# fwilliams/point-cloud-utils

Hardware: AMD Instinct MI355X
Metric: query-points/s, Chamfer 1M-vs-1M fp32 (higher is better)
Workload: dtype f32

## Files before the change

### point_cloud_utils_amd/csrc/search.h

```cpp
#pragma once
#include "pcu_types.h"
#include "grid.h"
#include "reduce.h"

namespace pcu {

template <typename T>
struct SearchArgs {
    const GridParams<T>* gp;
    const Pt4<T>* ref;
    const T* ref_xyz;
    const unsigned* cell_start;
    const Pt4<T>* qsorted;
    const T* q_xyz; const int* q_idx;
    const int* ref_idx;
    int lean;
    const int* qlist;
    const int* qcount_dev;
    int nq;
    int R;
    const int* qlist2; const int* qcount2_dev; int R2;
    unsigned n_ref;
    unsigned lane_max_cand;
    float skew_far;
// ... 286 lines not shown
        if (!active || outside) return;
    }

    const int ccx = grid_cell(g, 0, q.x), ccy = grid_cell(g, 1, q.y), ccz = grid_cell(g, 2, q.z);
    const int x0 = max(ccx - 1, 0), x1 = min(ccx + 1, Gx - 1);
    const int y0 = max(ccy - 1, 0), y1 = min(ccy + 1, Gy - 1);
    const int z0 = max(ccz - 1, 0), z1 = min(ccz + 1, Gz - 1);

    T bd[K];
    int bi[K];
#pragma unroll
    for (int i = 0; i < K; ++i) { bd[i] = Limits<T>::max_v; bi[i] = 0x7fffffff; }
    bool tie = false;

    unsigned rs[9], re[9];
#pragma unroll
    for (int j = 0; j < 9; ++j) {
        const int cy = ccy + kRowOy[j], cz = ccz + kRowOz[j];
        const bool ok = cy >= 0 && cy < Gy && cz >= 0 && cz < Gz;
        const int lo = row_run_lo(Gx, grid_row(Gy, ok ? cy : ccy, ok ? cz : ccz), x0, x1);
        rs[j] = a.cell_start[lo];
        const unsigned e = a.cell_start[lo + (x1 - x0 + 1)];
        re[j] = ok ? e : rs[j];
    }
    constexpr int kGroup = 4;
    const char* const base = reinterpret_cast<const char*>(a.ref);
    const unsigned sentinel = a.n_ref;
    unsigned total = 0;
#pragma unroll
    for (int j = 0; j < 9; ++j) total += re[j] - rs[j];
    const bool defer = total > a.lane_max_cand;
    T rlb[9];
    row_lower_bounds(g, q, ccy, ccz, rlb);
    constexpr int kBuf = K > 1 ? PCU_KBUF : 1;
    __shared__ T s_bd[kBuf][kBlock];
    __shared__ int s_bi[kBuf][kBlock];
    const int tid = threadIdx.x;
    int cnt = 0;
    auto flush = [&]() {
        int mx = cnt;
#pragma unroll
        for (int o = 32; o > 0; o >>= 1) mx = max(mx, __shfl_xor(mx, o, 64));
        for (int i = 0; i < mx; ++i)
            if (i < cnt) offer<T, K>(s_bd[i][tid], s_bi[i][tid], bd, bi, tie);
        cnt = 0;
    };
#pragma unroll
    for (int j = 0; j < 9; ++j) {
        if (K > 1 && __any(cnt >= kBuf / 2)) flush();
        const unsigned e = (defer || bd[K - 1] < rlb[j]) ? rs[j] : re[j];
        auto load_group = [&](unsigned p, Pt4<T> (&c)[kGroup]) {
#pragma unroll
            for (int u = 0; u < kGroup; ++u) {
                const unsigned idx = (p + u < e) ? p + u : sentinel;
                c[u] = *reinterpret_cast<const Pt4<T>*>(base + (size_t)(idx * (unsigned)sizeof(Pt4<T>)));
            }
        };
        auto eval_group = [&](const Pt4<T> (&c)[kGroup]) {
            if (K == 1) {
#pragma unroll
                for (int u = 0; u < kGroup; ++u) offer<T, K>(dist2(q, c[u]), (int)c[u].idx, bd, bi, tie);
            } else {
#pragma unroll
                for (int u = 0; u < kGroup; ++u) {
                    const T d = dist2(q, c[u]);
                    tie = tie || (d == bd[K - 1]);
                    if (d < bd[K - 1]) { s_bd[cnt][tid] = d; s_bi[cnt][tid] = (int)c[u].idx; ++cnt; }
                }
                if (__any(cnt > kBuf - kGroup)) flush();
            }
        };
        if (K > 1) {
            unsigned p = rs[j];
            if (p < e) {
                Pt4<T> ca[kGroup], cb[kGroup];
                load_group(p, ca);
                for (;;) {
                    p += kGroup;
                    load_group(p < e ? p : sentinel, cb);
                    eval_group(ca);
                    if (!(p < e)) break;
                    p += kGroup;
                    load_group(p < e ? p : sentinel, ca);
                    eval_group(cb);
                    if (!(p < e)) break;
                }
            }
        } else {
            for (unsigned p = rs[j]; p < e; p += kGroup) {
                Pt4<T> c[kGroup];
                load_group(p, c);
                eval_group(c);
            }
        }
    }
    if (K > 1) flush();

    finish_lane<T, K>(a, g, q, qpos, x0, x1, y0, y1, z0, z1, bd, bi, tie, true, defer);
}

__device__ __forceinline__ int cell_of_query(const GridParams<float>& g, const int axis, const float v) {
    const float t = (v - g.org[axis]) * g.inv_h;
    return (int)__builtin_amdgcn_fmed3f(t, 0.f, (float)(g.G[axis] - 1));
}
__device__ __forceinline__ int cell_of_query(const GridParams<double>& g, const int axis, const double v) { return grid_cell(g, axis, v); }
template <typename T> struct K1Group { static constexpr int n = 4; };
struct __attribute__((packed, aligned(4))) CellStart4 { unsigned v[4]; };
typedef float f32x2 __attribute__((ext_vector_type(2)));
__device__ __forceinline__ float min4(float a, float b, float c, float d) { return __builtin_fminf(__builtin_fminf(__builtin_fminf(a, b), c), d); }
__device__ __forceinline__ double min4(double a, double b, double c, double d) { return __builtin_fmin(__builtin_fmin(a, b), __builtin_fmin(c, d)); }

__device__ __forceinline__ unsigned lb_pack(float lb) { return __float_as_uint(lb) >> 16; }
__device__ __forceinline__ unsigned lb_pack(double lb) { const double v = lb * (1.0 - 1e-6); return __float_as_uint((float)(v < 1e38 ? v : 1e38)) >> 16; }
template <typename T> __device__ __forceinline__ T lb_unpack(unsigned b) { return (T)__uint_as_float(b << 16); }


template <typename T> struct __attribute__((packed, aligned(4))) Group12 { T v[12]; };
template <unsigned REC> __device__ __forceinline__ unsigned rec_bytes(unsigned i) {
    static_assert(REC == 12u || REC == 24u || REC == 16u || REC == 32u, "record sizes of the candidate streams");
    if (REC == 16u) return i << 4;
    if (REC == 32u) return i << 5;
    unsigned r; const unsigned t = REC == 12u ? i << 2 : i << 3;
    if (REC == 12u) asm("v_lshl_add_u32 %0, %1, 3, %2" : "=v"(r) : "v"(i), "v"(t));
    else asm("v_lshl_add_u32 %0, %1, 4, %2" : "=v"(r) : "v"(i), "v"(t));
    return r;
}
__device__ __forceinline__ unsigned mad24(unsigned a, unsigned b, unsigned c) { unsigned r; asm("v_mad_u32_u24 %0, %1, %2, %3" : "=v"(r) : "v"(a), "v"(b), "v"(c)); return r; }

template <typename T> struct GroupEval;
template <> struct GroupEval<float> {
    static constexpr unsigned kRec = 12u;
    typedef Group12<float> Raw;
    static __device__ __forceinline__ Raw load(const char* base, unsigned off) { return *reinterpret_cast<const Raw*>(base + (size_t)off); }
    static __device__ __forceinline__ void dists(const Raw& g, const Pt4<float>& q, float (&d)[4]) {
        const f32x2 qxy = {q.x, q.y}, qzx = {q.z, q.x}, qyz = {q.y, q.z};
        f32x2 p0 = qxy - f32x2{g.v[0], g.v[1]}, p1 = qzx - f32x2{g.v[2], g.v[3]}, p2 = qyz - f32x2{g.v[4], g.v[5]};
        f32x2 p3 = qxy - f32x2{g.v[6], g.v[7]}, p4 = qzx - f32x2{g.v[8], g.v[9]}, p5 = qyz - f32x2{g.v[10], g.v[11]};
        p0 = p0 * p0; p1 = p1 * p1; p2 = p2 * p2; p3 = p3 * p3; p4 = p4 * p4; p5 = p5 * p5;
        d[0] = (p0.x + p0.y) + p1.x; d[1] = (p1.y + p2.x) + p2.y; d[2] = (p3.x + p3.y) + p4.x; d[3] = (p4.y + p5.x) + p5.y;
    }
};
template <> struct GroupEval<double> {
    static constexpr unsigned kRec = 24u;
    typedef Group12<double> Raw;
    static __device__ __forceinline__ Raw load(const char* base, unsigned off) { return *reinterpret_cast<const Raw*>(base + (size_t)off); }
    static __device__ __forceinline__ void dists(const Raw& g, const Pt4<double>& q, double (&d)[4]) {
#pragma unroll
        for (int u = 0; u < 4; ++u) { const double dx = q.x - g.v[3 * u], dy = q.y - g.v[3 * u + 1], dz = q.z - g.v[3 * u + 2]; d[u] = ((dx * dx) + (dy * dy)) + (dz * dz); }
    }
};
template <typename T> struct BitsOf;
template <> struct BitsOf<float> { typedef unsigned type; static __device__ __forceinline__ unsigned of(float v) { return __float_as_uint(v); } static __device__ __forceinline__ float back(unsigned b) { return __uint_as_float(b); } };
template <> struct BitsOf<double> { typedef unsigned long long type; static __device__ __forceinline__ unsigned long long of(double v) { return (unsigned long long)__double_as_longlong(v); } static __device__ __forceinline__ double back(unsigned long long b) { return __longlong_as_double((long long)b); } };
template <typename T, bool EARLY, int FUSE>
__device__ __forceinline__ void search1_flat_body(const SearchArgs<T>& a, const int nq_arg, const int bid, const int nblk, bool& f_ok, T& f_v, long long& f_key) {
    typedef GroupEval<T> GE;
    __shared__ uint2 s_rng[8][kBlock];
    const int per = nblk >> 3;
    const int vb = (bid & 7) * per + (bid >> 3);
    const int tid = threadIdx.x;
    const int nq = a.qcount_dev ? *a.qcount_dev : nq_arg;
    if (vb * kBlock >= nq) return;
    const GridParams<T> g = uniform_params(*a.gp);
    if (const int hl = index_not_ready(a, g)) { if (vb == 0 && tid == 0) a.skew_flag[kLargeFlag] = hl; return; }
    const float ssq = uniform((float)g.sumsq);
    if (a.skew_limit > 0.f && (ssq > a.skew_limit || ssq < a.skew_lo)) { if (vb == 0 && tid == 0) *a.skew_flag = ssq > a.skew_far ? 2 : 1; return; }
    const int t = vb * kBlock + tid;
    if (t >= nq) return;
    constexpr bool valid = true;
    auto query_pos = [&]() { return a.qlist ? a.qlist[t] : t; };
    Pt4<T> q;
    {
        struct __attribute__((packed, aligned(4))) Q3 { T v[3]; };
        const Q3 c = *reinterpret_cast<const Q3*>(a.q_xyz + 3 * (size_t)query_pos());
        q.x = c.v[0]; q.y = c.v[1]; q.z = c.v[2];
        q.idx = 0;
    }
    static_assert(FUSE != FUSE_ARGMAX, "fused arg-max calls take the value-only program (FUSE_MAXVAL)");
    constexpr bool VALUE_ONLY = FUSE == FUSE_SUM || FUSE == FUSE_MAXVAL;
    const int Gx = g.G[0], Gy = g.G[1], Gz = g.G[2];
    const int ccx = cell_of_query(g, 0, q.x), ccy = cell_of_query(g, 1, q.y), ccz = cell_of_query(g, 2, q.z);
    constexpr unsigned kRec = GE::kRec;
    constexpr int kG = K1Group<T>::n;
    const char* const base = reinterpret_cast<const char*>(a.ref_xyz);
    const unsigned cand_cap = a.lane_max_cand < 65535u ? a.lane_max_cand : 65535u;
    T best = Limits<T>::max_v;
    unsigned boff = 0xffffffffu, toff = 0xffffffffu;
    bool tie = false, tie2 = false;
#define PCU_K1_EVAL(RAW, OFF)                                                                                \
    {                                                                                                        \
        T d_[4]; GE::dists((RAW), q, d_);                                                                    \
        const T m_ = min4(d_[0], d_[1], d_[2], d_[3]);                                                       \
        const bool eq_ = m_ == best, lt_ = m_ < best;                                                        \
        tie2 = !lt_ && (tie2 || (tie && eq_));                                                               \
        tie = !lt_ && (tie || eq_);                                                                          \
        toff = eq_ ? (OFF) : toff;                                                                           \
        best = lt_ ? m_ : best;                                                                              \
        boff = lt_ ? (OFF) : boff;                                                                           \
    }
    const bool hasxl = ccx > 0, hasxh = ccx < Gx - 1;
    const bool odd0 = ((ccy ^ ccz) & 1) != 0, zodd = (ccz & 1) != 0;
    const bool hasA = (odd0 && hasxh) || (!odd0 && hasxl), hasB = (odd0 && hasxl) || (!odd0 && hasxh);
    const unsigned Gx4 = (unsigned)Gx << 2;
    const unsigned xe4 = (unsigned)ccx << 2, xo4 = (unsigned)(Gx - 1 - ccx) << 2;
    const unsigned xS4 = odd0 ? xo4 : xe4, xR4 = odd0 ? xe4 : xo4;
    const int yS = zodd ? Gy - 1 - ccy : ccy, sS = zodd ? -1 : 1;
    const int row0 = (int)mad24((unsigned)ccz, (unsigned)Gy, (unsigned)yS);
    const int flip = (Gy - 1 - yS) - yS;
    const int rowM = row0 + flip - Gy, rowP = row0 + flip + Gy;
    const bool okyM = ccy > 0, okyP = ccy < Gy - 1, okzM = ccz > 0, okzP = ccz < Gz - 1;
    const char* const tbase = reinterpret_cast<const char*>(a.cell_start) - 4;
    auto row_table = [&](int j, bool& ok) {
        const int oy = kRowOy[j], oz = kRowOz[j];
        ok = (oy == 0 || (oy < 0 ? okyM : okyP)) && (oz == 0 || (oz < 0 ? okzM : okzP));
        const int rr = oz == 0 ? row0 + oy * sS : (oz < 0 ? rowM : rowP) - oy * sS;
        const unsigned row = (unsigned)(ok ? rr : row0);
        return *reinterpret_cast<const CellStart4*>(tbase + (size_t)(__umul24(row, Gx4) + (((oy + oz) & 1) == 0 ? xS4 : xR4)));
    };
    bool okj[9];
    CellStart4 tb[9];
    tb[0] = row_table(0, okj[0]);
    if (EARLY) {
#pragma unroll
        for (int j = 1; j < 9; ++j) tb[j] = row_table(j, okj[j]);
    }
    const unsigned c_s = hasA ? tb[0].v[0] : tb[0].v[1], c_e = hasB ? tb[0].v[3] : tb[0].v[2];
    const unsigned cnt0 = c_e - c_s;
    bool defer = cnt0 > cand_cap;
    {
        const unsigned o0 = rec_bytes<kRec>(c_s);
        const unsigned o1 = (defer || !valid) ? o0 : rec_bytes<kRec>(c_e);
        for (unsigned off = o0; off < o1; off += (unsigned)kG * kRec) { const typename GE::Raw raw = GE::load(base, off); PCU_K1_EVAL(raw, off) }
    }
    if (!EARLY) {
#pragma unroll
        for (int j = 1; j < 9; ++j) tb[j] = row_table(j, okj[j]);
    }
    const T shrink = (T)1 - (T)4 * Limits<T>::eps;
    T mxl = q.x - face_below(g, 0, ccx); mxl = mxl > (T)0 ? mxl * shrink : (T)0;
    T mxh = face_above(g, 0, ccx) - q.x; mxh = mxh > (T)0 ? mxh * shrink : (T)0;
    const T mxl2 = mxl * mxl, mxh2 = mxh * mxh;
    const T mA2 = odd0 ? mxh2 : mxl2, mB2 = odd0 ? mxl2 : mxh2;
    T my2[3], mz2[3];
    {
        T m;
        my2[0] = (T)0; mz2[0] = (T)0;
        m = q.y - face_below(g, 1, ccy); m = m > (T)0 ? m * shrink : (T)0; my2[1] = m * m;
        m = face_above(g, 1, ccy) - q.y; m = m > (T)0 ? m * shrink : (T)0; my2[2] = m * m;
        m = q.z - face_below(g, 2, ccz); m = m > (T)0 ? m * shrink : (T)0; mz2[1] = m * m;
        m = face_above(g, 2, ccz) - q.z; m = m > (T)0 ? m * shrink : (T)0; mz2[2] = m * m;
    }
    unsigned total = cnt0;
    int n = 0;
#pragma unroll
    for (int j = 1; j < 9; ++j) {
        const int oy = kRowOy[j], oz = kRowOz[j];
        const T ry = my2[oy == 0 ? 0 : (oy < 0 ? 1 : 2)], rz = mz2[oz == 0 ? 0 : (oz < 0 ? 1 : 2)];
        const bool same = ((oy + oz) & 1) == 0;
        const T mF2 = same ? mA2 : mB2, mL2 = same ? mB2 : mA2;
        const bool hasF = same ? hasA : hasB, hasL = same ? hasB : hasA;
        const T rlb = oy == 0 ? rz : (oz == 0 ? ry : ry + rz);
        const T bF = oy == 0 ? mF2 + rz : (oz == 0 ? mF2 + ry : (mF2 + ry) + rz), bL = oy == 0 ? mL2 + rz : (oz == 0 ? mL2 + ry : (mL2 + ry) + rz);
        const bool cutF = !hasF || best < bF, cutL = !hasL || best < bL;
        const unsigned s_run = cutF ? tb[j].v[1] : tb[j].v[0], e_run = cutL ? tb[j].v[2] : tb[j].v[3];
        const bool take = okj[j] && !defer && !(best < rlb) && e_run > s_run;
        s_rng[n][tid] = make_uint2(rec_bytes<kRec>(s_run), ((e_run - s_run) << 16) | lb_pack(rlb));
        n += take ? 1 : 0;
        total += take ? e_run - s_run : 0u;
    }
    if (total > cand_cap) { defer = true; n = 0; }
    const int own = tid;
    int r = 0;
    unsigned off = 0, end = 0;
    bool live = false;
    auto next_run = [&]() {
        live = false;
        while (r < n) {
            const uint2 e = s_rng[r][own];
            ++r;
            if (!(best < lb_unpack<T>(e.y & 0xffffu))) { off = e.x; end = e.x + __umul24(e.y >> 16, kRec); live = true; break; }
        }
    };
    next_run();
    const unsigned sent_off = a.n_ref * kRec;
#ifndef PCU_ADOPT_T
#define PCU_ADOPT_T 3
#endif
    if (VALUE_ONLY) {
        constexpr int kAdoptCap = 160;
        constexpr int kOwn = PCU_ADOPT_T;
        typedef typename BitsOf<T>::type Bits;
        __shared__ unsigned s_aitem[kBlock / 64][kAdoptCap];
        __shared__ Bits s_abest[kBlock / 64][64];
        const int lane_ = tid & 63, wave_ = tid >> 6;
        constexpr unsigned kStep = (unsigned)kG * kRec;
        if (live) {
            typename GE::Raw g0 = GE::load(base, off);
#pragma unroll
            for (int it = 0; it < kOwn; ++it) {
                const unsigned coff = off;
                off += kStep;
                if (off >= end) next_run();
                typename GE::Raw g1;
                if (it + 1 < kOwn) g1 = GE::load(base, live ? off : sent_off);
                PCU_K1_EVAL(g0, coff)
                if (!live) break;
                if (it + 1 < kOwn) g0 = g1;
            }
        }
        if (__ballot(true) == ~0ull && a.n_ref < (1u << 26)) {
            unsigned c = 0;
            if (live) {
                c = (end - off + kStep - 1u) / kStep;
                for (int rr = r; rr < n; ++rr) { const uint2 e = s_rng[rr][own]; if (!(best < lb_unpack<T>(e.y & 0xffffu))) c += ((e.y >> 16) + (unsigned)kG - 1u) / (unsigned)kG; }
            }
            unsigned inc = c;
#pragma unroll
            for (int o = 1; o < 64; o <<= 1) { const unsigned u = (unsigned)__shfl_up((int)inc, o, 64); if (lane_ >= o) inc += u; }
            const unsigned W = (unsigned)__shfl((int)inc, 63, 64);
            if (W != 0u && W <= (unsigned)kAdoptCap) {
                unsigned slot = inc - c;
                const unsigned tag = (unsigned)lane_ << 26;
                if (c) {
                    for (unsigned o = off; o < end; o += kStep) { s_aitem[wave_][slot] = (o / kRec) | tag; ++slot; }
                    for (int rr = r; rr < n; ++rr) {
                        const uint2 e = s_rng[rr][own];
                        if (!(best < lb_unpack<T>(e.y & 0xffffu))) {
                            const unsigned r0 = e.x / kRec, r1 = r0 + (e.y >> 16);
                            for (unsigned o = r0; o < r1; o += (unsigned)kG) { s_aitem[wave_][slot] = o | tag; ++slot; }
                        }
                    }
                }
                s_abest[wave_][lane_] = BitsOf<T>::of(best);
                __builtin_amdgcn_fence(__ATOMIC_RELEASE, "wavefront");
                __builtin_amdgcn_wave_barrier();
                __builtin_amdgcn_fence(__ATOMIC_ACQUIRE, "wavefront");
                for (unsigned wb = 0; wb < W; wb += 64u) {
                    const unsigned w_ = wb + (unsigned)lane_;
                    const bool in_ = w_ < W;
                    const unsigned it_ = in_ ? s_aitem[wave_][in_ ? w_ : 0u] : 0u;
                    const int ql = in_ ? (int)(it_ >> 26) : lane_;
                    const typename GE::Raw g1 = GE::load(base, in_ ? rec_bytes<kRec>(it_ & 0x03ffffffu) : sent_off);
                    Pt4<T> qq; qq.x = __shfl(q.x, ql, 64); qq.y = __shfl(q.y, ql, 64); qq.z = __shfl(q.z, ql, 64); qq.idx = 0;
                    T d_[4]; GE::dists(g1, qq, d_);
                    const T m_ = min4(d_[0], d_[1], d_[2], d_[3]);
                    if (in_) atomicMin(&s_abest[wave_][ql], BitsOf<T>::of(m_));
                }
                __builtin_amdgcn_fence(__ATOMIC_RELEASE, "wavefront");
                __builtin_amdgcn_wave_barrier();
                __builtin_amdgcn_fence(__ATOMIC_ACQUIRE, "wavefront");
                best = BitsOf<T>::back(s_abest[wave_][lane_]);
                live = false;
            }
        }
    }
    if (live) {
        typename GE::Raw ga = GE::load(base, off), gb;
        for (;;) {
            unsigned coff = off;
            off += (unsigned)kG * kRec;
            if (off >= end) next_run();
            gb = GE::load(base, live ? off : sent_off);
            PCU_K1_EVAL(ga, coff)
            if (!live) break;
            coff = off;
            off += (unsigned)kG * kRec;
            if (off >= end) next_run();
            ga = GE::load(base, live ? off : sent_off);
            PCU_K1_EVAL(gb, coff)
            if (!live) break;
        }
    }
    T lb;
    {
        const T smax = g.slack[0] > g.slack[1] ? (g.slack[0] > g.slack[2] ? g.slack[0] : g.slack[2]) : (g.slack[1] > g.slack[2] ? g.slack[1] : g.slack[2]);
        const T mag = ((fabs(g.org[0]) + fabs(g.org[1])) + fabs(g.org[2])) + (T)(Gx + Gy + Gz + 3) * g.h + smax;
        const T hq = (g.h - (T)2 * smax) - (T)16 * Limits<T>::eps * mag;
        const T hs = hq > (T)0 ? hq * shrink : (T)0;
        lb = hs * hs;
    }
    if (__ballot(valid && !defer && !(best < lb)) != 0ull) {
        const int cx0 = max(ccx - 1, 0), cx1 = min(ccx + 1, Gx - 1);
        const int cy0 = max(ccy - 1, 0), cy1 = min(ccy + 1, Gy - 1), cz0 = max(ccz - 1, 0), cz1 = min(ccz + 1, Gz - 1);
        lb = face_lower_bound_inner(g, q.x, q.y, q.z, cx0, cx1, cy0, cy1, cz0, cz1);
        unsigned long long todo = __ballot(valid && !defer && !(best < lb));
        if (todo && __popcll(todo) <= 4 && __ballot(true) == ~0ull) {
            const int lane_ = tid & 63;
            while (todo) {
                const int l = __ffsll((long long)todo) - 1;
                todo &= todo - 1;
                Pt4<T> sq;
                sq.x = __shfl(q.x, l, 64); sq.y = __shfl(q.y, l, 64); sq.z = __shfl(q.z, l, 64); sq.idx = 0;
                const int scx = grid_cell(g, 0, sq.x), scy = grid_cell(g, 1, sq.y), scz = grid_cell(g, 2, sq.z);
                const int bx0 = max(scx - 2, 0), bx1 = min(scx + 2, Gx - 1), by0 = max(scy - 2, 0), by1 = min(scy + 2, Gy - 1);
                const int bz0 = max(scz - 2, 0), bz1 = min(scz + 2, Gz - 1);
                const int ny_ = by1 - by0 + 1, nrows = ny_ * (bz1 - bz0 + 1);
                T wbest = Limits<T>::max_v; unsigned wboff = 0xffffffffu, wtoff = 0xffffffffu; bool wtie = false, wtie2 = false;
                if ((lane_ >> 1) < nrows) {
                    const int r_ = lane_ >> 1;
                    const unsigned lo = (unsigned)row_run_lo(Gx, grid_row(Gy, by0 + r_ % ny_, bz0 + r_ / ny_), bx0, bx1);
                    const unsigned rs_ = a.cell_start[lo], re_ = a.cell_start[lo + (unsigned)(bx1 - bx0 + 1)];
                    const unsigned mid = rs_ + (((re_ - rs_ + 1u) >> 1) + 3u) / 4u * 4u;
                    const unsigned s_ = ((lane_ & 1) ? min(mid, re_) : rs_) * kRec, e_ = ((lane_ & 1) ? re_ : min(mid, re_)) * kRec;
                    for (unsigned off_ = s_; off_ < e_; off_ += (unsigned)kG * kRec) {
                        T d_[4]; GE::dists(GE::load(base, off_), sq, d_);
                        if (!(lane_ & 1)) {
#pragma unroll
                            for (int u = 1; u < 4; ++u) d_[u] = off_ + (unsigned)u * kRec >= e_ ? (T)INFINITY : d_[u];
                        }
                        const T m_ = min4(d_[0], d_[1], d_[2], d_[3]);
                        const bool eq_ = m_ == wbest, lt_ = m_ < wbest;
                        if (!VALUE_ONLY) { wtie2 = !lt_ && (wtie2 || (wtie && eq_)); wtie = !lt_ && (wtie || eq_); wtoff = eq_ ? off_ : wtoff; wboff = lt_ ? off_ : wboff; }
                        wbest = lt_ ? m_ : wbest;
                    }
                }
                T mn = wbest;
#pragma unroll
                for (int o = 32; o > 0; o >>= 1) { const T ot = __shfl_xor(mn, o, 64); mn = ot < mn ? ot : mn; }
                const T lb2 = face_lower_bound_inner(g, sq.x, sq.y, sq.z, bx0, bx1, by0, by1, bz0, bz1);
                if (VALUE_ONLY) {
                    if (lane_ == l) { best = mn; lb = lb2; }
                    continue;
                }
                const unsigned long long eqm = __ballot(wbest == mn && wboff != 0xffffffffu);
                const int wl = eqm ? __ffsll((long long)eqm) - 1 : 0;
                const bool many = __popcll(eqm) > 1;
                const unsigned rb = (unsigned)__shfl((int)wboff, wl, 64), rt = many ? (unsigned)__shfl((int)wboff, 63 - __clzll((long long)eqm), 64) : (unsigned)__shfl((int)wtoff, wl, 64);
                const bool holds = wbest == mn && wboff != 0xffffffffu;
                const bool any_tie = __ballot(holds && wtie) != 0ull, any_tie2 = __ballot(holds && wtie2) != 0ull;
                const bool rtie = many || any_tie, rtie2 = (many && __popcll(eqm) > 2) || any_tie2 || (many && any_tie);
                if (lane_ == l) {
                    best = mn; lb = lb2; boff = eqm ? rb : 0xffffffffu; toff = rt; tie = rtie; tie2 = rtie2;
                }
            }
        }
    }
#undef PCU_K1_EVAL
    int bi[1] = {0x7fffffff};
    auto which = [&](unsigned goff, int& hits, unsigned& rec_off) {
        T d_[4]; GE::dists(GE::load(base, goff), q, d_);
        hits = 0; rec_off = 0xffffffffu;
#pragma unroll
        for (int u = kG - 1; u >= 0; --u) { const bool eq = d_[u] == best; hits += eq ? 1 : 0; rec_off = eq ? goff + (unsigned)u * kRec : rec_off; }
    };
    auto row_id = [&](unsigned rec_off) -> int { return a.ref_idx[rec_off / kRec]; };
    if (!VALUE_ONLY && boff != 0xffffffffu) {
        int hits; unsigned ro;
        which(boff, hits, ro);
        if (ro != 0xffffffffu) bi[0] = row_id(ro);
        if (hits > 1) { tie = true; tie2 = true; }
        if (tie && !tie2) {
            int h2; unsigned ro2;
            which(toff, h2, ro2);
            if (h2 == 1 && ro2 == ro) tie = false;
        }
    }
    const int qpos = query_pos();
    if (FUSE == FUSE_NONE) {
        if (defer) { wave_append(valid, qpos, a.ties, a.n_ties); return; }
        const bool certified = valid && best < lb;
        if (certified) {
            const size_t o = (size_t)a.q_idx[qpos] * (size_t)a.kreq;
            const bool found = bi[0] != 0x7fffffff;
            a.out_i[o] = found ? (long long)bi[0] : -1ll;
            a.out_d[o] = found ? (a.squared ? best : sqrt(best)) : (T)-1;
        }
        const int us = wave_append(valid && !certified, qpos, a.unresolved, a.n_unresolved);
        if (us >= 0 && a.ubound) a.ubound[us] = best;
        wave_append(certified && tie, qpos, a.ties, a.n_ties);
        return;
    }
    if (defer) {
        wave_append(valid, qpos, a.ties, a.n_ties);
        return;
    }
    const bool certified = valid && best < lb;
    const int us = wave_append(valid && !certified, qpos, a.unresolved, a.n_unresolved);
    if (us >= 0 && a.ubound) a.ubound[us] = best;
    f_ok = certified;
    f_v = a.squared ? best : sqrt(best);
    if (FUSE == FUSE_MAXVAL) f_key = ((long long)a.q_idx[qpos] << 32) | kKeyUnresolved | (long long)qpos;
}
#ifndef PCU_RUNS_MINW
#define PCU_RUNS_MINW 1
#endif
template <typename T, int K>
__global__ __launch_bounds__(kBlock, (sizeof(T) == 4 && K == 16) ? PCU_RUNS_MINW : 1) void k_search_runs(const SearchArgs<T> a) {
    static_assert(K > 1, "k = 1 has k_search1_flat");
    const int per = (int)(gridDim.x >> 3);
    const int vb = (int)(blockIdx.x & 7) * per + (int)(blockIdx.x >> 3);
    const int tid = threadIdx.x;
    const int t = vb * kBlock + tid;
    const int nq = a.qcount_dev ? *a.qcount_dev : a.nq;
    const GridParams<T>& g = *a.gp;
    if (t >= nq) return;
    const int qpos = a.qlist ? a.qlist[t] : t;
    const Pt4<T> q = a.qsorted[qpos];
    if (const int hl = index_not_ready(a, g)) { if (t == 0) a.skew_flag[kLargeFlag] = hl; return; }
    if (a.skew_limit > 0.f && ((float)g.sumsq > a.skew_limit || (float)g.sumsq < a.skew_lo)) { if (t == 0) *a.skew_flag = (float)g.sumsq > a.skew_far ? 2 : 1; return; }
    const int Gx = g.G[0], Gy = g.G[1], Gz = g.G[2];
    const int ccx = cell_of_query(g, 0, q.x), ccy = cell_of_query(g, 1, q.y), ccz = cell_of_query(g, 2, q.z);

    T bd[K]; int bi[K];
#pragma unroll
    for (int i = 0; i < K; ++i) { bd[i] = Limits<T>::max_v; bi[i] = 0x7fffffff; }
    bool tie = false;
    constexpr int kBuf = PCU_KBUF;
    constexpr int kGroup = 4;
    __shared__ T s_bd[kBuf][kBlock];
    __shared__ int s_bi[kBuf][kBlock];
    __shared__ uint2 s_rng[8][kBlock];
    int cnt = 0;
    auto flush = [&]() {
        int mx = cnt;
#pragma unroll
        for (int o = 32; o > 0; o >>= 1) mx = max(mx, __shfl_xor(mx, o, 64));
        for (int i = 0; i < mx; ++i)
            if (i < cnt) offer<T, K>(s_bd[i][tid], s_bi[i][tid], bd, bi, tie);
        cnt = 0;
    };
    const unsigned sentinel = a.n_ref;
    struct Grp { Pt4<T> c[kGroup]; unsigned p, e; };
    const char* const base = reinterpret_cast<const char*>(a.ref);
    auto load_group = [&](unsigned p, unsigned e, Grp& gr) {
        gr.p = p; gr.e = e;
#pragma unroll
        for (int u = 0; u < kGroup; ++u) {
            const unsigned idx = (p + u < e) ? p + u : sentinel;
            gr.c[u] = *reinterpret_cast<const Pt4<T>*>(base + (size_t)(idx * (unsigned)sizeof(Pt4<T>)));
        }
    };
    auto eval_group = [&](const Grp& gr) {
#pragma unroll
        for (int u = 0; u < kGroup; ++u) {
            const T d = dist2(q, gr.c[u]);
            tie = tie || (d == bd[K - 1]);
            if (d < bd[K - 1]) { s_bd[cnt][tid] = d; s_bi[cnt][tid] = (int)gr.c[u].idx; ++cnt; }
        }
        if (__any(cnt > kBuf - kGroup)) flush();
    };

    const bool hasxl = ccx > 0, hasxh = ccx < Gx - 1;
    const bool odd0 = ((ccy ^ ccz) & 1) != 0, zodd = (ccz & 1) != 0;
    const bool hasA = (odd0 && hasxh) || (!odd0 && hasxl), hasB = (odd0 && hasxl) || (!odd0 && hasxh);
    const unsigned Gx4 = (unsigned)Gx << 2;
    const unsigned xe4 = (unsigned)ccx << 2, xo4 = (unsigned)(Gx - 1 - ccx) << 2;
    const unsigned xS4 = odd0 ? xo4 : xe4, xR4 = odd0 ? xe4 : xo4;
    const int yS = zodd ? Gy - 1 - ccy : ccy, sS = zodd ? -1 : 1;
    const int row0 = (int)mad24((unsigned)ccz, (unsigned)Gy, (unsigned)yS);
    const int flip = (Gy - 1 - yS) - yS;
    const int rowM = row0 + flip - Gy, rowP = row0 + flip + Gy;
    const bool okyM = ccy > 0, okyP = ccy < Gy - 1, okzM = ccz > 0, okzP = ccz < Gz - 1;
    const char* const tbase = reinterpret_cast<const char*>(a.cell_start) - 4;
    bool okj[9];
    CellStart4 tb[9];
    auto row_table = [&](int j) {
        const int oy = kRowOy[j], oz = kRowOz[j];
        okj[j] = (oy == 0 || (oy < 0 ? okyM : okyP)) && (oz == 0 || (oz < 0 ? okzM : okzP));
        const int rr = oz == 0 ? row0 + oy * sS : (oz < 0 ? rowM : rowP) - oy * sS;
        const unsigned row = (unsigned)(okj[j] ? rr : row0);
        tb[j] = *reinterpret_cast<const CellStart4*>(tbase + (size_t)(__umul24(row, Gx4) + (((oy + oz) & 1) == 0 ? xS4 : xR4)));
    };
    row_table(0);
    const unsigned c_s = hasA ? tb[0].v[0] : tb[0].v[1], c_e = hasB ? tb[0].v[3] : tb[0].v[2];
    const unsigned cnt0 = c_e - c_s;
    const unsigned cand_cap = a.lane_max_cand < 65535u ? a.lane_max_cand : 65535u;
    bool defer = cnt0 > cand_cap;
    if (!defer && cnt0 > 0u) {
        unsigned p = c_s;
        Grp ca, cb;
        load_group(p, c_e, ca);
        for (;;) {
            p += kGroup;
            load_group(p, c_e, cb);
            eval_group(ca);
            if (!(p < c_e)) break;
            p += kGroup;
            load_group(p, c_e, ca);
            eval_group(cb);
            if (!(p < c_e)) break;
        }
    }
#pragma unroll
    for (int j = 1; j < 9; ++j) row_table(j);
    if (__any(cnt > 0)) flush();
    const T shrink = (T)1 - (T)4 * Limits<T>::eps;
    T mxl = q.x - face_below(g, 0, ccx); mxl = mxl > (T)0 ? mxl * shrink : (T)0;
    T mxh = face_above(g, 0, ccx) - q.x; mxh = mxh > (T)0 ? mxh * shrink : (T)0;
    const T mxl2 = mxl * mxl, mxh2 = mxh * mxh;
    const T mA2 = odd0 ? mxh2 : mxl2, mB2 = odd0 ? mxl2 : mxh2;
    T my2[3], mz2[3];
    {
        T m;
        my2[0] = (T)0; mz2[0] = (T)0;
        m = q.y - face_below(g, 1, ccy); m = m > (T)0 ? m * shrink : (T)0; my2[1] = m * m;
        m = face_above(g, 1, ccy) - q.y; m = m > (T)0 ? m * shrink : (T)0; my2[2] = m * m;
        m = q.z - face_below(g, 2, ccz); m = m > (T)0 ? m * shrink : (T)0; mz2[1] = m * m;
        m = face_above(g, 2, ccz) - q.z; m = m > (T)0 ? m * shrink : (T)0; mz2[2] = m * m;
    }
    unsigned total = cnt0;
    int n = 0;
    {
        const T kth = bd[K - 1];
#pragma unroll
        for (int j = 1; j < 9; ++j) {
            const int oy = kRowOy[j], oz = kRowOz[j];
            const T ry = my2[oy == 0 ? 0 : (oy < 0 ? 1 : 2)], rz = mz2[oz == 0 ? 0 : (oz < 0 ? 1 : 2)];
            const bool same = ((oy + oz) & 1) == 0;
            const T mF2 = same ? mA2 : mB2, mL2 = same ? mB2 : mA2;
            const bool hasF = same ? hasA : hasB, hasL = same ? hasB : hasA;
// ... 337 lines not shown
```

### scratch/replay_adopt.py

```python
import numpy as np
rng=np.random.default_rng(1)
n=200000
P=rng.random((n,3)); Q=rng.random((n,3))
G=int(round((n/2)**(1/3))); h=1.0/G
def cells(X): return np.minimum((X/h).astype(int),G-1)
cp=cells(P)
key=(cp[:,2]*G+cp[:,1])*G+cp[:,0]
order=np.argsort(key,kind='stable'); P=P[order]; key=key[order]
start=np.searchsorted(key,np.arange(G*G*G+1))
cq=cells(Q); kq=(cq[:,2]*G+cq[:,1])*G+cq[:,0]; oq=np.argsort(kq,kind='stable'); Q=Q[oq]; cq=cq[oq]
rows=[(0,0),(-1,0),(1,0),(0,-1),(0,1),(-1,-1),(1,-1),(-1,1),(1,1)]
def lane(qi):
    q=Q[qi]; cx,cy,cz=cq[qi]
    def run(cy_,cz_,x0,x1):
        if cy_<0 or cy_>=G or cz_<0 or cz_>=G: return None
        x0=max(x0,0); x1=min(x1,G-1)
        if x1<x0: return None
        b=(cz_*G+cy_)*G
        return start[b+x0], start[b+x1+1]
    s,e=run(cy,cz,cx-1,cx+1)
    best=np.inf; g0=0; p=s
    while p<e:
        d=((P[p:p+4]-q)**2).sum(1); best=min(best,d.min()); p+=4; g0+=1
    mxl=q[0]-cx*h; mxh=(cx+1)*h-q[0]
    my={-1:q[1]-cy*h,0:0.0,1:(cy+1)*h-q[1]}; mz={-1:q[2]-cz*h,0:0.0,1:(cz+1)*h-q[2]}
    ent=[]
    for (oy,oz) in rows[1:]:
        rlb=my[oy]**2+mz[oz]**2
        if best<rlb: continue
        x0=cx-1 if not (best<mxl**2+rlb) else cx
        x1=cx+1 if not (best<mxh**2+rlb) else cx
        r=run(cy+oy,cz+oz,x0,x1)
        if r is None or r[1]<=r[0]: continue
        ent.append((rlb,r))
    return q,g0,best,ent
def simulate(qi,T):
    q,g0,best,ent=lane(qi)
    done=0; i=0; p=None; e=None
    while done<T:
        if p is None or p>=e:
            while i<len(ent) and best<ent[i][0]: i+=1
            if i>=len(ent): return g0,done,0
            p,e=ent[i][1]; i+=1
        d=((P[p:p+4]-q)**2).sum(1); best=min(best,d.min()); p+=4; done+=1
    rem=0
    if p is not None and p<e: rem+=(e-p+3)//4
    for j in range(i,len(ent)):
        if not (best<ent[j][0]): rem+=(ent[j][1][1]-ent[j][1][0]+3)//4
    return g0,done,rem
nw=40; base=64*1000
for T in (1000,2,3,4,5,6):
    res=np.array([simulate(base+i,T) for i in range(64*nw)])
    own=res[:,1].reshape(nw,64); rem=res[:,2].reshape(nw,64)
    trips=own.max(1)+np.ceil(rem.sum(1)/64)
    print("T=%4d  own max/wave %.2f  W mean %.1f (max %d)  dealt trips %.2f  total outer trips %.2f"%(T,own.max(1).mean(),rem.sum(1).mean(),rem.sum(1).max(),np.ceil(rem.sum(1)/64).mean(),trips.mean()))
```

Measured before the change: 16.77 billion.

## Cap centre-row scan at two groups and defer remainder to wave-shared adoption

The centre row scan is limited to two groups loaded together, and any remaining centre-row records become the lane's first live run, so they go into the wave-level adoption/dealing pool rather than being walked serially per lane. The inclusive prefix sum over the wave now uses DPP row-shift and row-broadcast instructions in place of a shuffle-based loop, and readlane replaces a shuffle for the total. Some loops are marked nounroll, and the query-list pointer is reloaded as a uniform value late in the kernel. The aim is less divergence among lanes with large centre cells, at the cost of more adoption work and a larger share of waves exceeding the adoption cap.

```diff
diff --git a/point_cloud_utils_amd/csrc/search.h b/point_cloud_utils_amd/csrc/search.h
--- a/point_cloud_utils_amd/csrc/search.h
+++ b/point_cloud_utils_amd/csrc/search.h
@@ -462,6 +462,15 @@
 template <typename T> struct BitsOf;
 template <> struct BitsOf<float> { typedef unsigned type; static __device__ __forceinline__ unsigned of(float v) { return __float_as_uint(v); } static __device__ __forceinline__ float back(unsigned b) { return __uint_as_float(b); } };
 template <> struct BitsOf<double> { typedef unsigned long long type; static __device__ __forceinline__ unsigned long long of(double v) { return (unsigned long long)__double_as_longlong(v); } static __device__ __forceinline__ double back(unsigned long long b) { return __longlong_as_double((long long)b); } };
+__device__ __forceinline__ unsigned wave_scan_add(unsigned x) {
+    x += (unsigned)__builtin_amdgcn_update_dpp(0, (int)x, 0x111, 0xf, 0xf, false);
+    x += (unsigned)__builtin_amdgcn_update_dpp(0, (int)x, 0x112, 0xf, 0xf, false);
+    x += (unsigned)__builtin_amdgcn_update_dpp(0, (int)x, 0x114, 0xf, 0xf, false);
+    x += (unsigned)__builtin_amdgcn_update_dpp(0, (int)x, 0x118, 0xf, 0xf, false);
+    x += (unsigned)__builtin_amdgcn_update_dpp(0, (int)x, 0x142, 0xa, 0xf, false);
+    x += (unsigned)__builtin_amdgcn_update_dpp(0, (int)x, 0x143, 0xc, 0xf, false);
+    return x;
+}
 template <typename T, bool EARLY, int FUSE>
 __device__ __forceinline__ void search1_flat_body(const SearchArgs<T>& a, const int nq_arg, const int bid, const int nblk, bool& f_ok, T& f_v, long long& f_key) {
     typedef GroupEval<T> GE;
@@ -537,10 +546,17 @@
     const unsigned c_s = hasA ? tb[0].v[0] : tb[0].v[1], c_e = hasB ? tb[0].v[3] : tb[0].v[2];
     const unsigned cnt0 = c_e - c_s;
     bool defer = cnt0 > cand_cap;
+    unsigned c_rem = 0, c_end = 0;
     {
+        constexpr unsigned kStep0 = (unsigned)kG * kRec;
         const unsigned o0 = rec_bytes<kRec>(c_s);
         const unsigned o1 = (defer || !valid) ? o0 : rec_bytes<kRec>(c_e);
-        for (unsigned off = o0; off < o1; off += (unsigned)kG * kRec) { const typename GE::Raw raw = GE::load(base, off); PCU_K1_EVAL(raw, off) }
+        const bool has1 = o0 + kStep0 < o1;
+        const typename GE::Raw g0 = GE::load(base, o0);
+        const typename GE::Raw g1 = GE::load(base, has1 ? o0 + kStep0 : o0);
+        PCU_K1_EVAL(g0, o0)
+        if (has1) PCU_K1_EVAL(g1, o0 + kStep0)
+        c_rem = o0 + 2u * kStep0; c_end = o1;
     }
     if (!EARLY) {
 #pragma unroll
@@ -591,7 +607,8 @@
             if (!(best < lb_unpack<T>(e.y & 0xffffu))) { off = e.x; end = e.x + __umul24(e.y >> 16, kRec); live = true; break; }
         }
     };
-    next_run();
+    if (c_rem < c_end && !defer) { off = c_rem; end = c_end; live = true; }
+    else next_run();
     const unsigned sent_off = a.n_ref * kRec;
 #ifndef PCU_ADOPT_T
 #define PCU_ADOPT_T 3
@@ -622,21 +639,23 @@
             unsigned c = 0;
             if (live) {
                 c = (end - off + kStep - 1u) / kStep;
+#pragma nounroll
                 for (int rr = r; rr < n; ++rr) { const uint2 e = s_rng[rr][own]; if (!(best < lb_unpack<T>(e.y & 0xffffu))) c += ((e.y >> 16) + (unsigned)kG - 1u) / (unsigned)kG; }
             }
-            unsigned inc = c;
-#pragma unroll
-            for (int o = 1; o < 64; o <<= 1) { const unsigned u = (unsigned)__shfl_up((int)inc, o, 64); if (lane_ >= o) inc += u; }
-            const unsigned W = (unsigned)__shfl((int)inc, 63, 64);
+            const unsigned inc = wave_scan_add(c);
+            const unsigned W = (unsigned)__builtin_amdgcn_readlane((int)inc, 63);
             if (W != 0u && W <= (unsigned)kAdoptCap) {
                 unsigned slot = inc - c;
                 const unsigned tag = (unsigned)lane_ << 26;
                 if (c) {
-                    for (unsigned o = off; o < end; o += kStep) { s_aitem[wave_][slot] = (o / kRec) | tag; ++slot; }
+#pragma nounroll
+                    for (unsigned o = off / kRec, o1 = end / kRec; o < o1; o += (unsigned)kG) { s_aitem[wave_][slot] = o | tag; ++slot; }
+#pragma nounroll
                     for (int rr = r; rr < n; ++rr) {
                         const uint2 e = s_rng[rr][own];
                         if (!(best < lb_unpack<T>(e.y & 0xffffu))) {
                             const unsigned r0 = e.x / kRec, r1 = r0 + (e.y >> 16);
+#pragma nounroll
                             for (unsigned o = r0; o < r1; o += (unsigned)kG) { s_aitem[wave_][slot] = o | tag; ++slot; }
                         }
                     }
@@ -765,7 +784,8 @@
             if (h2 == 1 && ro2 == ro) tie = false;
         }
     }
-    const int qpos = query_pos();
+    const int* const qlist_late = reinterpret_cast<const int*>(uniform((unsigned long long)reinterpret_cast<size_t>(a.qlist)));
+    const int qpos = qlist_late ? qlist_late[t] : t;
     if (FUSE == FUSE_NONE) {
         if (defer) { wave_append(valid, qpos, a.ties, a.n_ties); return; }
         const bool certified = valid && best < lb;
diff --git a/scratch/replay_adopt.py b/scratch/replay_adopt.py
--- a/scratch/replay_adopt.py
+++ b/scratch/replay_adopt.py
@@ -1,56 +1,101 @@
+import sys
 import numpy as np
-rng=np.random.default_rng(1)
-n=200000
-P=rng.random((n,3)); Q=rng.random((n,3))
-G=int(round((n/2)**(1/3))); h=1.0/G
-def cells(X): return np.minimum((X/h).astype(int),G-1)
-cp=cells(P)
-key=(cp[:,2]*G+cp[:,1])*G+cp[:,0]
-order=np.argsort(key,kind='stable'); P=P[order]; key=key[order]
-start=np.searchsorted(key,np.arange(G*G*G+1))
-cq=cells(Q); kq=(cq[:,2]*G+cq[:,1])*G+cq[:,0]; oq=np.argsort(kq,kind='stable'); Q=Q[oq]; cq=cq[oq]
-rows=[(0,0),(-1,0),(1,0),(0,-1),(0,1),(-1,-1),(1,-1),(-1,1),(1,1)]
-def lane(qi):
-    q=Q[qi]; cx,cy,cz=cq[qi]
-    def run(cy_,cz_,x0,x1):
-        if cy_<0 or cy_>=G or cz_<0 or cz_>=G: return None
-        x0=max(x0,0); x1=min(x1,G-1)
-        if x1<x0: return None
-        b=(cz_*G+cy_)*G
-        return start[b+x0], start[b+x1+1]
-    s,e=run(cy,cz,cx-1,cx+1)
-    best=np.inf; g0=0; p=s
-    while p<e:
-        d=((P[p:p+4]-q)**2).sum(1); best=min(best,d.min()); p+=4; g0+=1
-    mxl=q[0]-cx*h; mxh=(cx+1)*h-q[0]
-    my={-1:q[1]-cy*h,0:0.0,1:(cy+1)*h-q[1]}; mz={-1:q[2]-cz*h,0:0.0,1:(cz+1)*h-q[2]}
-    ent=[]
-    for (oy,oz) in rows[1:]:
-        rlb=my[oy]**2+mz[oz]**2
-        if best<rlb: continue
-        x0=cx-1 if not (best<mxl**2+rlb) else cx
-        x1=cx+1 if not (best<mxh**2+rlb) else cx
-        r=run(cy+oy,cz+oz,x0,x1)
-        if r is None or r[1]<=r[0]: continue
-        ent.append((rlb,r))
-    return q,g0,best,ent
-def simulate(qi,T):
-    q,g0,best,ent=lane(qi)
-    done=0; i=0; p=None; e=None
-    while done<T:
-        if p is None or p>=e:
-            while i<len(ent) and best<ent[i][0]: i+=1
-            if i>=len(ent): return g0,done,0
-            p,e=ent[i][1]; i+=1
-        d=((P[p:p+4]-q)**2).sum(1); best=min(best,d.min()); p+=4; done+=1
-    rem=0
-    if p is not None and p<e: rem+=(e-p+3)//4
-    for j in range(i,len(ent)):
-        if not (best<ent[j][0]): rem+=(ent[j][1][1]-ent[j][1][0]+3)//4
-    return g0,done,rem
-nw=40; base=64*1000
-for T in (1000,2,3,4,5,6):
-    res=np.array([simulate(base+i,T) for i in range(64*nw)])
-    own=res[:,1].reshape(nw,64); rem=res[:,2].reshape(nw,64)
-    trips=own.max(1)+np.ceil(rem.sum(1)/64)
-    print("T=%4d  own max/wave %.2f  W mean %.1f (max %d)  dealt trips %.2f  total outer trips %.2f"%(T,own.max(1).mean(),rem.sum(1).mean(),rem.sum(1).max(),np.ceil(rem.sum(1)/64).mean(),trips.mean()))
+
+ROWS = [(0, 0), (-1, 0), (1, 0), (0, -1), (0, 1), (-1, -1), (1, -1), (-1, 1), (1, 1)]
+CAP = 160
+
+
+class Replay:
+    def __init__(self, P, Q):
+        P = np.asarray(P, np.float64); Q = np.asarray(Q, np.float64)
+        lo = np.minimum(P.min(0), Q.min(0)); hi = np.maximum(P.max(0), Q.max(0))
+        n = len(P)
+        self.G = G = max(1, int(round((n / 2) ** (1 / 3)))); self.h = h = float((hi - lo).max()) / G * (1 + 1e-9); self.lo = lo
+        cp = self.cells(P)
+        key = (cp[:, 2] * G + cp[:, 1]) * G + cp[:, 0]
+        order = np.argsort(key, kind='stable'); self.P = P[order]; key = key[order]
+        self.start = np.searchsorted(key, np.arange(G * G * G + 1))
+        cq = self.cells(Q); kq = (cq[:, 2] * G + cq[:, 1]) * G + cq[:, 0]; oq = np.argsort(kq, kind='stable')
+        self.Q = Q[oq]; self.cq = cq[oq]
+
+    def cells(self, X):
+        return np.clip(((X - self.lo) / self.h).astype(int), 0, self.G - 1)
+
+    def lane(self, qi, centre):
+        G, h, P, start = self.G, self.h, self.P, self.start
+        q = self.Q[qi]; cx, cy, cz = self.cq[qi]; rel = q - self.lo
+
+        def run(cy_, cz_, x0, x1):
+            if cy_ < 0 or cy_ >= G or cz_ < 0 or cz_ >= G: return None
+            x0 = max(x0, 0); x1 = min(x1, G - 1)
+            if x1 < x0: return None
+            b = (cz_ * G + cy_) * G
+            return start[b + x0], start[b + x1 + 1]
+        s, e = run(cy, cz, cx - 1, cx + 1)
+        best = np.inf; g0 = 0; p = s
+        while p < e and g0 < centre:
+            d = ((P[p:p + 4] - q) ** 2).sum(1); best = min(best, d.min()); p += 4; g0 += 1
+        ent = [(0.0, (p, e))] if p < e else []
+        mxl = rel[0] - cx * h; mxh = (cx + 1) * h - rel[0]
+        my = {-1: rel[1] - cy * h, 0: 0.0, 1: (cy + 1) * h - rel[1]}; mz = {-1: rel[2] - cz * h, 0: 0.0, 1: (cz + 1) * h - rel[2]}
+        for (oy, oz) in ROWS[1:]:
+            rlb = my[oy] ** 2 + mz[oz] ** 2
+            if best < rlb: continue
+            x0 = cx - 1 if not (best < mxl ** 2 + rlb) else cx
+            x1 = cx + 1 if not (best < mxh ** 2 + rlb) else cx
+            r = run(cy + oy, cz + oz, x0, x1)
+            if r is None or r[1] <= r[0]: continue
+            ent.append((rlb, r))
+        return q, g0, best, ent
+
+    def simulate(self, qi, T, centre):
+        q, g0, best, ent = self.lane(qi, centre)
+        P = self.P
+        done = 0; i = 0; p = None; e = None
+        while done < T:
+            if p is None or p >= e:
+                while i < len(ent) and best < ent[i][0]: i += 1
+                if i >= len(ent): return g0, done, 0
+                p, e = ent[i][1]; i += 1
+            d = ((P[p:p + 4] - q) ** 2).sum(1); best = min(best, d.min()); p += 4; done += 1
+        rem = 0
+        if p is not None and p < e: rem += (e - p + 3) // 4
+        for j in range(i, len(ent)):
+            if not (best < ent[j][0]): rem += (ent[j][1][1] - ent[j][1][0] + 3) // 4
+        return g0, done, rem
+
+    def outcomes(self, T=3, centre=2):
+        nq = len(self.Q); nfull = nq // 64
+        W = np.array([sum(self.simulate(w * 64 + l, T, centre)[2] for l in range(64)) for w in range(nfull)])
+        return int((W == 0).sum()), int(((W > 0) & (W <= CAP)).sum()), int((W > CAP).sum()), nq % 64
+
+
+def path_inputs(dtype=np.float32):
+    rng = np.random.default_rng(20260)
+    a = rng.random((20_000, 3)).astype(dtype)
+    u1, u2 = rng.random((30_037, 3)).astype(dtype), rng.random((40_000, 3)).astype(dtype)
+
+    def slab(n_u, n_p):
+        u = rng.random((n_u, 3)); pl = rng.random((n_p, 3)); pl[:, 2] = 0.5 + 1e-3 * (pl[:, 2] - 0.5)
+        return np.concatenate([u, pl]).astype(dtype)
+    return {"self": (a, a.copy()), "uniform": (u1, u2), "slab": (slab(20_000, 12_011), slab(20_000, 12_000))}
+
+
+if __name__ == "__main__":
+    if len(sys.argv) > 1 and sys.argv[1] == "paths":
+        for name, (x, y) in path_inputs().items():
+            for tag, (qq, pp) in (("x->y", (x, y)), ("y->x", (y, x))):
+                z, w, o, part = Replay(pp, qq).outcomes()
+                print("%-8s %s  waves: nothing owed %d, within the cap %d, over the cap %d; lanes in a partial last wave %d" % (name, tag, z, w, o, part))
+        sys.exit(0)
+    rng = np.random.default_rng(1)
+    n = 200000
+    R = Replay(rng.random((n, 3)), rng.random((n, 3)))
+    nw = 40; base = 64 * 1000
+    for centre in (1000, 2):
+        for T in (1000, 2, 3, 4):
+            res = np.array([R.simulate(base + i, T, centre) for i in range(64 * nw)])
+            cen = res[:, 0].reshape(nw, 64); own = res[:, 1].reshape(nw, 64); rem = res[:, 2].reshape(nw, 64)
+            trips = cen.max(1) + own.max(1) + np.ceil(rem.sum(1) / 64)
+            print("centre cap %4d T=%4d  centre max/wave %.2f  own max/wave %.2f  W mean %.1f (max %d, over the cap %d of %d)  dealt trips %.2f  total trips %.2f" % (
+                centre, T, cen.max(1).mean(), own.max(1).mean(), rem.sum(1).mean(), rem.sum(1).max(), (rem.sum(1) > CAP).sum(), nw, np.ceil(rem.sum(1) / 64).mean(), trips.mean()))
```

After: 17.04 billion (median of 6 runs). Within noise of the previous version (+1.6%).
